# EasyVision-Ton/VMG

Measured on AMD Instinct MI355X. Metric: LR-frames/s (train: forward+loss+backward+AdamW), VMG-REDS-few_levels 4x SR, higher is better.
Workload: dtype bf16; 1 GPU; VMG-REDS-few_levels train step, per-GPU batch 4x7x3x64x64 -> 4x SR (BASELINE configs[1]); global_batch=4, frames_per_clip=7, parallelism=dp1, launch=eager, recompute_chains=False, fp8_chains=False

## Files before the change

include/vmg_hip.h:

```cpp
#ifndef VMG_HIP_H
#define VMG_HIP_H

#include <stdint.h>

#ifdef __cplusplus
extern "C" {
#endif

#define VMG_F32 0
#define VMG_BF16 1

#define VMG_ACT_NONE 0
#define VMG_ACT_RELU 1
#define VMG_ACT_LRELU 2
#define VMG_ACT_GELU 3

#define VMG_CONV_GENERAL 0
#define VMG_CONV_KSPLIT 2
#define VMG_CONV_WS 3
#define VMG_CONV_LINEAR_WRES 4
#define VMG_CONV_WSTAT 6

const char* vmg_last_error(void);
int vmg_version(void);
// ... 150 lines not shown
                       int B, int D, int H, int W, int C, int heads, int wt, int sd, int sh, int sw, void* stream);
int64_t vmg_win3d_attn_bwd_ws_bytes(int B, int D, int H, int W, int heads, int wt);
int vmg_win3d_attn_bwd(int dtype, const void* q, const void* kv, const float* bq, const float* bkv, const float* table, const void* out,
                       const float* lse, const void* d_out, void* dq, void* dkv, float* dtable, float* dbq, float* dbkv, void* ws, int B, int D, int H, int W,
                       int C, int heads, int wt, int sd, int sh, int sw, void* stream);
int vmg_win3d_variant(int variant);

int vmg_maxpool_fwd(int dtype, const void* x, void* y, unsigned char* idx, int N, int H, int W, int C, int f, void* stream);
int vmg_maxpool_bwd(int dtype, const void* dy, const unsigned char* idx, void* dx, int N, int H, int W, int C, int f, void* stream);

int vmg_se_mlp_fwd(const float* m, const float* w1, const float* b1, const float* w2, const float* b2, float* pre, float* out, int G, int C,
                   int Hd, int Co, int act1, int mode, void* stream);
int vmg_se_mlp_bwd(const float* dout, const float* out, const float* m, const float* pre, const float* w1, const float* w2, float* dm,
                   float* dw1, float* db1, float* dw2, float* db2, float* ws, int G, int C, int Hd, int Co, int act1, int mode, float dm_scale,
                   int accumulate, void* stream);

int vmg_avgpool2_nhwc(int dtype, const void* x, void* y, int n, int h, int w, int c, void* stream);
int vmg_upsample2x_ac_fwd(const float* x, float* y, int n, int h, int w, int c, float scale, void* stream);
int vmg_upsample2x_ac_bwd(const float* dy, float* dx, int n, int h, int w, int c, float scale, void* stream);
int vmg_spy_operand_fwd(int dtype, const void* ref, const void* warped, const float* up, void* out, int64_t npix, void* stream);
int vmg_spy_operand_bwd(int dtype, const void* dx8, void* dwarped, float* dup, int64_t npix, void* stream);
int vmg_spy_flow_add(int dtype, const float* up, const void* res, float* out, int64_t n, void* stream);
int vmg_spy_prep(int dtype, const float* img, const float* mean, const float* stdv, void* out, int64_t n, int h, int w, void* stream);

int vmg_tile_accumulate(int dtype, const void* patch, float* E, float* Wt, int64_t planes, int ph, int pw, int EH, int EW, int oh, int ow,
                        int top, int bottom, int left, int right, void* stream);
int vmg_tile_finalize(const float* E, const float* Wt, float* out_f32, unsigned char* out_u8, int64_t n, void* stream);

int64_t vmg_frame_metrics_ws_bytes(int T, int H, int W);
int vmg_frame_metrics(const unsigned char* a, const int64_t* a_strides, const unsigned char* b, const int64_t* b_strides, int T, int H, int W,
// ... 54 lines not shown
```

vmg_amd/csrc/tab_ops.hip:

```cpp
#include "common.h"

namespace {

template <typename T>
struct V16 {
  static constexpr int N = 16 / sizeof(T);
  T v[N];
};

template <typename T, int VN>
__global__ __launch_bounds__(256) void group_reduce_kernel(const T* __restrict__ a, const T* __restrict__ b, const T* __restrict__ c3,
                                                           float* __restrict__ out, int G, long long R, int C, int mode, float scale,
                                                           int chunks) {
  struct alignas(sizeof(T) * VN) Vec { T v[VN]; };
  __shared__ float red[VN * 256];
  const int g = blockIdx.x / chunks, ck = blockIdx.x - g * chunks;
  const int tpr = C / VN;
  const int rpb = 256 / tpr;
  const int roff = threadIdx.x / tpr, cp = threadIdx.x - roff * tpr;
  const long long r0 = R * ck / chunks, r1 = R * (ck + 1) / chunks;
  float s[VN];
#pragma unroll
  for (int e = 0; e < VN; ++e) s[e] = 0.f;
  if (roff < rpb) {
    const long long base = (long long)g * R * C + VN * cp;
    constexpr int U = 4;
    for (long long r = r0 + roff; r < r1; r += (long long)U * rpb) {
      Vec va[U], vb[U], vc[U];
      bool ok[U];
#pragma unroll
      for (int u = 0; u < U; ++u) {
// ... 22 lines not shown
#pragma unroll
          for (int e = 0; e < VN; ++e) s[e] += to_f32(va[u].v[e]) * to_f32(vb[u].v[e]);
        }
      }
    }
  }
#pragma unroll
  for (int e = 0; e < VN; ++e) red[e * 256 + threadIdx.x] = s[e];
  __syncthreads();
  for (int c = threadIdx.x; c < C; c += 256) {
    const int cp2 = c / VN, e = c - cp2 * VN;
    float t = 0.f;
    for (int k = 0; k < rpb; ++k) t += red[e * 256 + k * tpr + cp2];
    out[((long long)g * chunks + ck) * C + c] = t;
  }
}

__global__ __launch_bounds__(256) void group_reduce_final_kernel(const float* __restrict__ partial, float* __restrict__ out, int G, int chunks, int width,
                                                                 float scale) {
  __shared__ float sm[16][17];
  const int slabs = (width + 15) >> 4;
  const int g = blockIdx.x / slabs, c = (blockIdx.x - g * slabs) * 16 + (threadIdx.x & 15);
  const int q = threadIdx.x >> 4;
  float t = 0.f;
  if (c < width) {
    const float* p = partial + (long long)g * chunks * width + c;
#pragma unroll 4
    for (int k = q; k < chunks; k += 16) t += p[(long long)k * width];
  }
  sm[q][threadIdx.x & 15] = t;
  __syncthreads();
  if (q == 0 && c < width) {
    float u = 0.f;
#pragma unroll
    for (int i = 0; i < 16; ++i) u += sm[i][threadIdx.x & 15];
    out[(long long)g * width + c] = u * scale;
  }
}

template <typename T, int VN>
__global__ __launch_bounds__(256) void group_reduce3_kernel(const T* __restrict__ a, const T* __restrict__ b0, const T* __restrict__ b1,
                                                            const T* __restrict__ b2, float* __restrict__ out, int G, long long R, int C,
                                                            float scale, int chunks) {
  struct alignas(sizeof(T) * VN) Vec { T v[VN]; };
  __shared__ float red[3 * VN * 256];
  const int g = blockIdx.x / chunks, ck = blockIdx.x - g * chunks;
  const int tpr = C / VN;
  const int rpb = 256 / tpr;
  const int roff = threadIdx.x / tpr, cp = threadIdx.x - roff * tpr;
  const long long r0 = R * ck / chunks, r1 = R * (ck + 1) / chunks;
  float s[3][VN];
#pragma unroll
  for (int k = 0; k < 3; ++k)
#pragma unroll
    for (int e = 0; e < VN; ++e) s[k][e] = 0.f;
  if (roff < rpb) {
    const long long base = (long long)g * R * C + VN * cp;
    for (long long r = r0 + roff; r < r1; r += rpb) {
      const long long o = base + r * C;
      const Vec va = *reinterpret_cast<const Vec*>(a + o);
      const Vec v0 = *reinterpret_cast<const Vec*>(b0 + o), v1 = *reinterpret_cast<const Vec*>(b1 + o), v2 = *reinterpret_cast<const Vec*>(b2 + o);
// ... 6 lines not shown
      }
    }
  }
#pragma unroll
  for (int k = 0; k < 3; ++k)
#pragma unroll
    for (int e = 0; e < VN; ++e) red[(k * VN + e) * 256 + threadIdx.x] = s[k][e];
  __syncthreads();
  for (int i = threadIdx.x; i < 3 * C; i += 256) {
    const int c = i / 3, k = i - 3 * c;
    const int cp2 = c / VN, e = c - cp2 * VN;
    float t = 0.f;
    for (int j = 0; j < rpb; ++j) t += red[(k * VN + e) * 256 + j * tpr + cp2];
    out[(((long long)g * chunks + ck) * C + c) * 3 + k] = t;
  }
}

enum { OP_CA_FWD = 0, OP_CA_BWD = 1, OP_MIX_FWD = 2, OP_MIX_BWD = 3, OP_GATE_FWD = 4, OP_GATE_BWD = 5, OP_AFFINE2 = 6, OP_SCALE = 7, OP_GATE_RES_FWD = 8, OP_GATE_RES_BWD = 9 };

template <typename T>
__global__ __launch_bounds__(256) void tab_ew_kernel(int op, const T* __restrict__ p0, const T* __restrict__ p1, const T* __restrict__ p2,
                                                     const float* __restrict__ coef, const float* __restrict__ add, float s,
                                                     T* __restrict__ o0, T* __restrict__ o1, T* __restrict__ o2, long long rows,
                                                     long long R, int C) {
  constexpr int VN = V16<T>::N;
  const int nvec = C / VN;
  const long long total = rows * nvec;
  for (long long i = blockIdx.x * 256LL + threadIdx.x; i < total; i += (long long)gridDim.x * 256) {
    const long long row = i / nvec;
    const int v = (int)(i - row * nvec);
// ... 246 lines not shown
  } else if (i < n1 + n2) {
    const int e = i - n1, o = e / Hd, j = e - o * Hd;
    for (int g = 0; g < G; ++g) s += dz2[(long long)g * Co + o] * se_act(pre[g * Hd + j], act1);
    dw2[e] = accumulate ? dw2[e] + s : s;
  } else if (i < n1 + n2 + Hd) {
    const int j = i - n1 - n2;
    for (int g = 0; g < G; ++g) s += dz1[g * Hd + j];
    db1[j] = accumulate ? db1[j] + s : s;
  } else if (i < n1 + n2 + Hd + Co) {
    const int o = i - n1 - n2 - Hd;
    for (int g = 0; g < G; ++g) s += dz2[(long long)g * Co + o];
    db2[o] = accumulate ? db2[o] + s : s;
  }
}

}

extern "C" int vmg_se_mlp_fwd(const float* m, const float* w1, const float* b1, const float* w2, const float* b2, float* pre, float* out, int G,
                              int C, int Hd, int Co, int act1, int mode, void* stream) {
  VMG_CHECK(m && w1 && w2 && pre && out && G > 0 && C > 0 && Hd > 0 && Co > 0, "se_mlp_fwd: bad arguments");
  VMG_CHECK((act1 == 1 || act1 == 3) && (mode == 0 || (mode == 1 && Co % 3 == 0)), "se_mlp_fwd: act1 is ReLU (1) or GELU (3); mode 1 needs Co = 3 * channels");
  VMG_CHECK((C + Hd) * 4 <= 64 * 1024, "se_mlp_fwd: C + Hd too large");
  hipLaunchKernelGGL(se_mlp_fwd_kernel, dim3(G), dim3(1024), (C + Hd) * 4, (hipStream_t)stream, m, w1, b1, w2, b2, pre, out, C, Hd, Co, act1, mode);
  VMG_LAUNCH_CHECK();
  return 0;
}

extern "C" int vmg_se_mlp_bwd(const float* dout, const float* out, const float* m, const float* pre, const float* w1, const float* w2, float* dm,
                              float* dw1, float* db1, float* dw2, float* db2, float* ws, int G, int C, int Hd, int Co, int act1, int mode,
                              float dm_scale, int accumulate, void* stream) {
// ... 83 lines not shown
  const int chunks = gr_chunks(G, R);
  VMG_CHECK((int64_t)G * chunks * C * 3 * (int64_t)sizeof(float) <= ws_bytes, "group_reduce3: workspace too small (vmg_group_reduce_ws_bytes)");
  hipStream_t st = (hipStream_t)stream;
  if (dtype == VMG_BF16)
    hipLaunchKernelGGL((group_reduce3_kernel<bf16, 8>), dim3(G * chunks), dim3(256), 0, st, (const bf16*)a, (const bf16*)b0, (const bf16*)b1,
                       (const bf16*)b2, ws, G, (long long)R, C, scale, chunks);
  else
    hipLaunchKernelGGL((group_reduce3_kernel<float, 4>), dim3(G * chunks), dim3(256), 0, st, (const float*)a, (const float*)b0, (const float*)b1,
                       (const float*)b2, ws, G, (long long)R, C, scale, chunks);
  VMG_LAUNCH_CHECK();
  hipLaunchKernelGGL(group_reduce_final_kernel, dim3(G * cdiv(3 * C, 16)), dim3(256), 0, st, (const float*)ws, out, G, chunks, 3 * C, scale);
  VMG_LAUNCH_CHECK();
  return 0;
}

extern "C" int vmg_tab_elementwise(int dtype, int op, const void* p0, const void* p1, const void* p2, const float* coef, const float* add,
                                   float s, void* o0, void* o1, void* o2, int64_t rows, int64_t R, int C, void* stream) {
  VMG_CHECK(dtype == VMG_F32 || dtype == VMG_BF16, "tab_elementwise: bad dtype");
  VMG_CHECK(op >= 0 && op <= 9 && p0 && o0 && rows > 0 && R > 0 && C > 0, "tab_elementwise: bad arguments");
  const int vn = dtype == VMG_BF16 ? 8 : 4;
  VMG_CHECK(C % vn == 0, "tab_elementwise: C must be a multiple of %d", vn);
  const long long total = rows * (C / vn);
  const int blocks = (int)(cdiv64(total, 256) > 8192 ? 8192 : cdiv64(total, 256));
  hipStream_t st = (hipStream_t)stream;
  if (dtype == VMG_BF16)
    hipLaunchKernelGGL(tab_ew_kernel<bf16>, dim3(blocks), dim3(256), 0, st, op, (const bf16*)p0, (const bf16*)p1, (const bf16*)p2, coef, add, s,
                       (bf16*)o0, (bf16*)o1, (bf16*)o2, (long long)rows, (long long)R, C);
  else
    hipLaunchKernelGGL(tab_ew_kernel<float>, dim3(blocks), dim3(256), 0, st, op, (const float*)p0, (const float*)p1, (const float*)p2, coef, add,
                       s, (float*)o0, (float*)o1, (float*)o2, (long long)rows, (long long)R, C);
// ... 4 lines not shown
```

vmg_amd/functional.py:

```python
from __future__ import annotations

from typing import List, Optional, Sequence

import torch

from . import hip
from . import kernels as K
from .hip import HipError

class _Fn(torch.autograd.Function):

    @classmethod
    def apply(cls, *args):
        return super(torch.autograd.Function, cls).apply(*args)


def _pad_to(n: int, m: int = 8) -> int:
    return (n + m - 1) // m * m


def choose_tiling(M: int, cout: int, ks: int, dtype: torch.dtype, src_ch: Optional[Sequence[int]] = None, pixel_shuffle: bool = False):
    if USE_WS and src_ch is not None and not pixel_shuffle:
        t = K.ws_eligible(cout, ks, dtype, src_ch)
        if t and M <= 16384 and cout in (112, 144):
# ... 57 lines not shown
            if planned and hit[0][1] == ver[1] and key not in self.volatile:
                self.volatile.add(key)
                self.stamp += 1
        ent = [ver, build(key, weight, buf), weight]
        if planned and key not in self.volatile and _from_param(ent):
            self.stamp += 1
        ents[key] = ent
        return ent[1]

    def clear(self):
        self.ents.clear()
        self.q8.clear()
        self.volatile.clear()
        self.decay = None
        self.stamp += 1

    def bump_epoch(self):
        self.epoch += 1

    def settled(self, since: int, with_repack: bool) -> bool:
        return self.stamp == since and self.vol.stamp == since and (not with_repack or self.stable.stamp == since)

    def _run_plan(self, st: _PlanState, wkey, member, reset_sig: bool = False):
        fresh = st.stamp != self.stamp or st.wkey != wkey
        if fresh:
            st.ents = [ent for key, ent in self.ents.items() if member(key, ent)]
            st.packs, st.stamp, st.wkey = [ent[1] for ent in st.ents], self.stamp, wkey
            if reset_sig:
                st.plan.sig = None
        if not st.packs:
# ... 1016 lines not shown
        axis, chunk, Cp, shape = ctx.cfg
        return K.morph_tokens_gather(g.contiguous(), axis, chunk, Cp, Cp), None, None, None, None


def morph_linear(x: torch.Tensor, weight: torch.Tensor, bias: Optional[torch.Tensor], axis: str, chunk: int, Cp: int) -> torch.Tensor:
    if K.morph_fused_ok(x, chunk, Cp):
        return _MorphLinear.apply(x, weight, bias, axis, chunk, Cp)
    tok = _MorphGather.apply(x, axis, chunk, Cp)
    if tok.shape[-1] != Cp:
        padded, tok = tok, tok[:, :Cp]
        tok._vmg_padded = padded
    t = linear(tok, weight, bias, act=hip.ACT_RELU, alpha=1.0 / Cp)
    return _MorphScatter.apply(t, axis, chunk, Cp, tuple(x.shape))


class _ChannelAttention(_Fn):

    @staticmethod
    def forward(ctx, r, x, w1, b1, w2, b2, s):
        r, x = r.contiguous(), x.contiguous()
        N, C = r.shape[0], r.shape[-1]
        R = r.numel() // (N * C)
        m = K.group_reduce(r, N, scale=1.0 / R)
        pre, g = K.se_mlp_forward(m, w1.flatten(1), b1, w2.flatten(1), b2, hip.ACT_RELU, 0)
        out = K.tab_elementwise(K.OP_CA_FWD, r, x, coef=g, s=s, G=N)
        ctx.s, ctx.R = s, R
        ctx.save_for_backward(r, g, m, pre, w1, w2)
        DEFERRED.claim(ctx, w1, b1, w2, b2)
        return out

    @staticmethod
    def backward(ctx, dy):
        r, g, m, pre, w1, w2 = ctx.saved_tensors
        s, R = ctx.s, ctx.R
        dy = dy.contiguous()
        N = r.shape[0]
        dg = K.group_reduce(dy, N, b=r, mode=1, scale=s)
        dm, dw1, db1, dw2, db2 = K.se_mlp_backward(dg, g, m, pre, w1.flatten(1), w2.flatten(1), hip.ACT_RELU, 0, 1.0 / R, into=DEFERRED.into(ctx))
        d_r, d_x = K.tab_elementwise(K.OP_CA_BWD, dy, coef=g, add=dm, s=s, G=N, nout=2)
        DEFERRED.done(ctx)
        if ctx.direct:
            return d_r, d_x, None, None, None, None, None
        return (d_r, d_x, dw1.reshape(w1.shape), db1, dw2.reshape(w2.shape), db2, None)


def channel_attention_residual(r, x, w1, b1, w2, b2, out_scale: float):
    return _ChannelAttention.apply(r, x, w1, b1, w2, b2, float(out_scale))

class _ResidualDropPath(_Fn):

    @staticmethod
    def forward(ctx, res, y, g, gb=None):
        out = K.tab_elementwise(K.OP_CA_FWD, y.contiguous(), res.contiguous(), coef=g, s=1.0, G=g.shape[0])
# ... 66 lines not shown
            mask.div_(keep)
        g = (mask * scale).expand(B, C).contiguous()
    else:
        g = torch.full((B, C), float(scale), dtype=torch.float32, device=y.device)
    return _ResidualDropPath.apply(res, y, g)



class _ReweightMix(_Fn):

    @staticmethod
    def forward(ctx, h, w, c, fc1w, fc1b, fc2w, fc2b):
        h, w, c = h.contiguous(), w.contiguous(), c.contiguous()
        B, C = h.shape[0], h.shape[-1]
        R = h.numel() // (B * C)
        m = K.group_reduce(h, B, b=w, c3=c, scale=1.0 / R)
        pre, a = K.se_mlp_forward(m, fc1w, fc1b, fc2w, fc2b, hip.ACT_GELU, 1)
        y = K.tab_elementwise(K.OP_MIX_FWD, h, w, c, coef=a, G=B)
        ctx.R = R
        ctx.save_for_backward(h, w, c, a, m, pre, fc1w, fc2w)
        DEFERRED.claim(ctx, fc1w, fc1b, fc2w, fc2b)
        return y

    @staticmethod
    def backward(ctx, dy):
        h, w, c, a, m, pre, fc1w, fc2w = ctx.saved_tensors
        R = ctx.R
        dy = dy.contiguous()
        B, C = h.shape[0], h.shape[-1]
        da = K.group_reduce3(dy, h, w, c, B).reshape(B, 3 * C)
        dm, dw1, db1, dw2, db2 = K.se_mlp_backward(da, a, m, pre, fc1w, fc2w, hip.ACT_GELU, 1, 1.0 / R, into=DEFERRED.into(ctx))
        dh, dw, dc = K.tab_elementwise(K.OP_MIX_BWD, dy, coef=a, add=dm, G=B, nout=3)
        DEFERRED.done(ctx)
        if ctx.direct:
            return dh, dw, dc, None, None, None, None
        return dh, dw, dc, dw1, db1, dw2, db2


def reweight_mix(h, w, c, fc1w, fc1b, fc2w, fc2b):
    return _ReweightMix.apply(h, w, c, fc1w, fc1b, fc2w, fc2b)


class _TanhGate(_Fn):

    @staticmethod
    def forward(ctx, x, y):
# ... 352 lines not shown
```

vmg_amd/hip.py:

```python
from __future__ import annotations

import ctypes
import os
from ctypes import POINTER, c_char_p, c_float, c_int, c_int64, c_void_p

import torch

HERE = os.path.dirname(os.path.abspath(__file__))
LIB_PATH = os.environ.get("VMG_HIP_LIB") or os.path.join(HERE, "libvmg_hip.so")

F32, BF16 = 0, 1
ACT_NONE, ACT_RELU, ACT_LRELU, ACT_GELU = 0, 1, 2, 3
CONV_GENERAL, CONV_KSPLIT, CONV_WS, CONV_LINEAR_WRES, CONV_WSTAT = 0, 2, 3, 4, 6


class HipError(RuntimeError):
    pass


class ConvDesc(ctypes.Structure):
    _fields_ = [
        ("dtype", c_int), ("ks", c_int), ("cout_tiles", c_int),
        ("N", c_int), ("H", c_int), ("W", c_int), ("Cout", c_int),
        ("nsrc", c_int),
# ... 79 lines not shown
    "vmg_win3d_variant": (c_int, [c_int]),
    "vmg_linear_wgrad2_multi": (c_int, [c_int, c_int, c_void_p, c_void_p, c_int64, c_int64, c_int, c_int64, c_int, c_void_p, c_int, c_int, c_int,
                                        c_void_p, c_void_p, c_void_p, c_int64, c_void_p]),
    "vmg_replay_build": (c_void_p, [c_void_p, c_void_p, c_void_p]),
    "vmg_replay_kernel_info": (c_int, [c_void_p, c_int, c_void_p, c_void_p, c_void_p, c_void_p]),
    "vmg_replay_run": (c_int, [c_void_p, c_int, c_int, c_void_p]),
    "vmg_replay_destroy": (None, [c_void_p]),
    "vmg_pack_entry_bytes": (c_int, []),
    "vmg_pack_entry": (c_int, [c_void_p, c_int, c_int, c_void_p, c_int, c_int, c_int, c_int, c_int, c_int, c_void_p, c_void_p, c_int, c_int, c_void_p,
                               c_int]),
    "vmg_pack_run": (c_int, [c_void_p, c_int, c_int, c_void_p]),
    "vmg_group_reduce3": (c_int, [c_int, c_void_p, c_void_p, c_void_p, c_void_p, c_void_p, c_int, c_int64, c_int, ctypes.c_float, c_void_p, c_int64, c_void_p]),
    "vmg_group_reduce_ws_bytes": (c_int64, []),
    "vmg_se_mlp_fwd": (c_int, [c_void_p] * 7 + [c_int] * 6 + [c_void_p]),
    "vmg_se_mlp_bwd": (c_int, [c_void_p] * 12 + [c_int] * 6 + [ctypes.c_float, c_int, c_void_p]),
    "vmg_maxpool_fwd": (c_int, [c_int, c_void_p, c_void_p, c_void_p, c_int, c_int, c_int, c_int, c_int, c_void_p]),
    "vmg_maxpool_bwd": (c_int, [c_int, c_void_p, c_void_p, c_void_p, c_int, c_int, c_int, c_int, c_int, c_void_p]),
    "vmg_avgpool2_nhwc": (c_int, [c_int, c_void_p, c_void_p, c_int, c_int, c_int, c_int, c_void_p]),
    "vmg_upsample2x_ac_fwd": (c_int, [c_void_p, c_void_p, c_int, c_int, c_int, c_int, c_float, c_void_p]),
    "vmg_upsample2x_ac_bwd": (c_int, [c_void_p, c_void_p, c_int, c_int, c_int, c_int, c_float, c_void_p]),
    "vmg_spy_operand_fwd": (c_int, [c_int, c_void_p, c_void_p, c_void_p, c_void_p, c_int64, c_void_p]),
    "vmg_spy_operand_bwd": (c_int, [c_int, c_void_p, c_void_p, c_void_p, c_int64, c_void_p]),
    "vmg_spy_flow_add": (c_int, [c_int, c_void_p, c_void_p, c_void_p, c_int64, c_void_p]),
    "vmg_spy_prep": (c_int, [c_int, c_void_p, c_void_p, c_void_p, c_void_p, c_int64, c_int, c_int, c_void_p]),
    "vmg_space_depth_ln_fwd": (c_int, [c_int, c_int, c_void_p, c_void_p, c_void_p, c_void_p, c_void_p, c_void_p, c_int, c_int, c_int, c_int, c_float, c_void_p]),
    "vmg_space_depth_ln_bwd": (c_int, [c_int, c_int, c_void_p, c_void_p, c_void_p, c_void_p, c_void_p, c_void_p, c_void_p, c_void_p, c_int, c_int, c_int, c_int,
                                       c_void_p, c_void_p]),
    "vmg_conv_wgrad_batched": (c_int, [c_int, c_int, c_int, POINTER(c_void_p), POINTER(c_void_p), c_int, c_int, c_int, c_int64, c_int,
                                       c_int64, c_int, c_void_p, c_int, c_int, c_int, c_void_p, c_float, c_void_p]),
    "vmg_warp_bilinear_fwd": (c_int, [c_int, c_void_p, c_void_p, c_void_p, c_int, c_int, c_int, c_int, c_void_p]),
# ... 110 lines not shown
```

vmg_amd/kernels.py:

```python
from __future__ import annotations

import ctypes
import os
import struct
from typing import Optional, Sequence, Tuple

import torch

from . import hip
from .hip import ConvDesc, HipError


def _intarr(v: Sequence[int]):
    return (ctypes.c_int * len(v))(*[int(x) for x in v])


def cout_tiles_for(cout: int, dtype: torch.dtype = torch.bfloat16, ks: int = 3) -> int:
    t = (cout + 15) // 16
    if t <= 1:
        return 1
    if ks == 7:
        return 2 if t == 2 else 4
    if t <= 4:
        return 4
# ... 996 lines not shown
        dm, ws = parts
        dw1, db1, dw2, db2 = into
        for t, n in zip(into, (Hd * C, Hd, Co * Hd, Co)):
            if t.dtype != torch.float32 or not t.is_contiguous() or t.numel() != n or not t.is_cuda:
                raise HipError("se_mlp: gradient buffers must be contiguous fp32 of the parameters' sizes")
    else:
        dm, ws, dw1, db1, dw2, db2 = parts
    hip.check(hip.lib().vmg_se_mlp_bwd(dout.data_ptr(), out.data_ptr(), m.data_ptr(), pre.data_ptr(), w1.data_ptr(), w2.data_ptr(), dm.data_ptr(),
                                       dw1.data_ptr(), db1.data_ptr(), dw2.data_ptr(), db2.data_ptr(), ws.data_ptr(), G, C, Hd, Co, act1, mode,
                                       float(dm_scale), 1 if into is not None else 0, hip.stream_ptr()), "vmg_se_mlp_bwd")
    if into is not None:
        return dm.view(G, C), dw1, db1, dw2, db2
    return dm.view(G, C), dw1.view(Hd, C), db1, dw2.view(Co, Hd), db2


class PackPlan:

    def __init__(self):
        self.sig, self.dev, self.n, self.blocks = None, None, 0, 0
        self.retired = []

    def run(self, packs: Sequence[PackedConv], reuse: bool = False):
        l = hip.lib()
        if reuse and self.sig is not None:
            hip.check(l.vmg_pack_run(self.dev.data_ptr(), self.n, self.blocks, hip.stream_ptr()), "vmg_pack_run")
            return
        packs = [p for p in packs if p.call is not None]
        if not packs:
            return
        sig = tuple((p.call[0], p.buf.data_ptr()) for p in packs)
# ... 153 lines not shown
```

Before: 599.4 LR-frames/s.

## Fuse pooled group reduction with SE-style gate MLP via last-block ticket

Adds fused forward and backward kernels that do the per-group pooled reduction and then, in the last-arriving workgroup per group (selected with an atomic ticket counter), finalize the reduction and run the small gate MLP. Backward also computes dm and, in a globally last workgroup, the weight and bias gradients. The aim is to replace several small kernel launches (reduce, final reduce, MLP fwd/bwd) with one launch per direction. The cost is serialized MLP work on one workgroup, plus atomics and fences that rely on the workspace counters being zeroed correctly.

```diff
diff --git a/include/vmg_hip.h b/include/vmg_hip.h
--- a/include/vmg_hip.h
+++ b/include/vmg_hip.h
@@ -188,6 +188,15 @@
 int vmg_se_mlp_bwd(const float* dout, const float* out, const float* m, const float* pre, const float* w1, const float* w2, float* dm,
                    float* dw1, float* db1, float* dw2, float* db2, float* ws, int G, int C, int Hd, int Co, int act1, int mode, float dm_scale,
                    int accumulate, void* stream);
+int64_t vmg_pooled_gate_ws_bytes(void);
+int64_t vmg_pooled_gate_counter_bytes(void);
+int vmg_pooled_gate_fwd(int dtype, const void* a, const void* b, const void* c3, const float* w1, const float* b1, const float* w2,
+                        const float* b2, float* m, float* pre, float* gate, int G, int64_t R, int C, int Hd, int Co, int act1, int mode,
+                        float scale, void* ws, int64_t ws_bytes, void* stream);
+int vmg_pooled_gate_bwd(int dtype, const void* dy, const void* b0, const void* b1, const void* b2, const float* gate, const float* m,
+                        const float* pre, const float* w1, const float* w2, float* dm, float* dw1, float* db1, float* dw2, float* db2,
+                        float* dz, int G, int64_t R, int C, int Hd, int Co, int act1, int mode, float scale, float dm_scale, int accumulate,
+                        void* ws, int64_t ws_bytes, void* stream);
 
 int vmg_avgpool2_nhwc(int dtype, const void* x, void* y, int n, int h, int w, int c, void* stream);
 int vmg_upsample2x_ac_fwd(const float* x, float* y, int n, int h, int w, int c, float scale, void* stream);
diff --git a/vmg_amd/csrc/tab_ops.hip b/vmg_amd/csrc/tab_ops.hip
--- a/vmg_amd/csrc/tab_ops.hip
+++ b/vmg_amd/csrc/tab_ops.hip
@@ -9,12 +9,10 @@
 };
 
 template <typename T, int VN>
-__global__ __launch_bounds__(256) void group_reduce_kernel(const T* __restrict__ a, const T* __restrict__ b, const T* __restrict__ c3,
-                                                           float* __restrict__ out, int G, long long R, int C, int mode, float scale,
-                                                           int chunks) {
+__device__ __forceinline__ void group_reduce_block(const T* __restrict__ a, const T* __restrict__ b, const T* __restrict__ c3,
+                                                   float* __restrict__ out, long long R, int C, int mode, int chunks, int g, int ck,
+                                                   float* __restrict__ red ) {
   struct alignas(sizeof(T) * VN) Vec { T v[VN]; };
-  __shared__ float red[VN * 256];
-  const int g = blockIdx.x / chunks, ck = blockIdx.x - g * chunks;
   const int tpr = C / VN;
   const int rpb = 256 / tpr;
   const int roff = threadIdx.x / tpr, cp = threadIdx.x - roff * tpr;
@@ -67,6 +65,15 @@
     for (int k = 0; k < rpb; ++k) t += red[e * 256 + k * tpr + cp2];
     out[((long long)g * chunks + ck) * C + c] = t;
   }
+}
+
+template <typename T, int VN>
+__global__ __launch_bounds__(256) void group_reduce_kernel(const T* __restrict__ a, const T* __restrict__ b, const T* __restrict__ c3,
+                                                           float* __restrict__ out, int G, long long R, int C, int mode, float scale,
+                                                           int chunks) {
+  __shared__ float red[VN * 256];
+  const int g = blockIdx.x / chunks, ck = blockIdx.x - g * chunks;
+  group_reduce_block<T, VN>(a, b, c3, out, R, C, mode, chunks, g, ck, red);
 }
 
 __global__ __launch_bounds__(256) void group_reduce_final_kernel(const float* __restrict__ partial, float* __restrict__ out, int G, int chunks, int width,
@@ -92,12 +99,10 @@
 }
 
 template <typename T, int VN>
-__global__ __launch_bounds__(256) void group_reduce3_kernel(const T* __restrict__ a, const T* __restrict__ b0, const T* __restrict__ b1,
-                                                            const T* __restrict__ b2, float* __restrict__ out, int G, long long R, int C,
-                                                            float scale, int chunks) {
+__device__ __forceinline__ void group_reduce3_block(const T* __restrict__ a, const T* __restrict__ b0, const T* __restrict__ b1,
+                                                    const T* __restrict__ b2, float* __restrict__ out, long long R, int C, int chunks, int g,
+                                                    int ck, float* __restrict__ red ) {
   struct alignas(sizeof(T) * VN) Vec { T v[VN]; };
-  __shared__ float red[3 * VN * 256];
-  const int g = blockIdx.x / chunks, ck = blockIdx.x - g * chunks;
   const int tpr = C / VN;
   const int rpb = 256 / tpr;
   const int roff = threadIdx.x / tpr, cp = threadIdx.x - roff * tpr;
@@ -134,6 +139,15 @@
     for (int j = 0; j < rpb; ++j) t += red[(k * VN + e) * 256 + j * tpr + cp2];
     out[(((long long)g * chunks + ck) * C + c) * 3 + k] = t;
   }
+}
+
+template <typename T, int VN>
+__global__ __launch_bounds__(256) void group_reduce3_kernel(const T* __restrict__ a, const T* __restrict__ b0, const T* __restrict__ b1,
+                                                            const T* __restrict__ b2, float* __restrict__ out, int G, long long R, int C,
+                                                            float scale, int chunks) {
+  __shared__ float red[3 * VN * 256];
+  const int g = blockIdx.x / chunks, ck = blockIdx.x - g * chunks;
+  group_reduce3_block<T, VN>(a, b0, b1, b2, out, R, C, chunks, g, ck, red);
 }
 
 enum { OP_CA_FWD = 0, OP_CA_BWD = 1, OP_MIX_FWD = 2, OP_MIX_BWD = 3, OP_GATE_FWD = 4, OP_GATE_BWD = 5, OP_AFFINE2 = 6, OP_SCALE = 7, OP_GATE_RES_FWD = 8, OP_GATE_RES_BWD = 9 };
@@ -410,6 +424,229 @@
   }
 }
 
+constexpr int PG_COUNTERS = 1024;
+constexpr int PG_FIN = 16 * 65;
+
+__device__ __forceinline__ bool pg_ticket(int* counter, int last) {
+  __shared__ int drew_last;
+  __threadfence();
+  __syncthreads();
+  if (threadIdx.x == 0) drew_last = atomicAdd(counter, 1) == last;
+  __syncthreads();
+  const bool r = drew_last != 0;
+  if (r) __threadfence();
+  return r;
+}
+
+__device__ __forceinline__ void pg_final(const float* part, int chunks, int width, float scale, float* fin, float* vec, float* outg) {
+  const int tid = threadIdx.x, q = tid >> 4, c4 = tid & 15;
+  for (int s0 = 0; s0 < width; s0 += 64) {
+    const int c = s0 + 4 * c4;
+    float t[4] = {0.f, 0.f, 0.f, 0.f};
+    if (c < width) {
+      for (int k0 = q; k0 < chunks; k0 += 128) {
+        float4 v[8];
+#pragma unroll
+        for (int u = 0; u < 8; ++u)
+          if (k0 + 16 * u < chunks) v[u] = *reinterpret_cast<const float4*>(part + (long long)(k0 + 16 * u) * width + c);
+#pragma unroll
+        for (int u = 0; u < 8; ++u)
+          if (k0 + 16 * u < chunks) { t[0] += v[u].x; t[1] += v[u].y; t[2] += v[u].z; t[3] += v[u].w; }
+      }
+    }
+#pragma unroll
+    for (int e = 0; e < 4; ++e) fin[q * 65 + 4 * c4 + e] = t[e];
+    __syncthreads();
+    if (tid < 64 && s0 + tid < width) {
+      float u = 0.f;
+#pragma unroll
+      for (int i = 0; i < 16; ++i) u += fin[i * 65 + tid];
+      u *= scale;
+      vec[s0 + tid] = u;
+      if (outg) outg[s0 + tid] = u;
+    }
+    __syncthreads();
+  }
+}
+
+template <typename F>
+__device__ __forceinline__ void pg_wave_dots(const float* x, int n, const float* __restrict__ W, int sx, int sj, int nj, F sink) {
+  constexpr int JB = 3, KM = 8;
+  const int lane = threadIdx.x & 63, wave = threadIdx.x >> 6;
+  for (int j0 = wave; j0 < nj; j0 += 4 * JB) {
+    float wv[JB][KM];
+#pragma unroll
+    for (int b = 0; b < JB; ++b)
+#pragma unroll
+      for (int k = 0; k < KM; ++k) {
+        const int j = j0 + 4 * b, i = lane + 64 * k;
+        wv[b][k] = (j < nj && i < n) ? W[(long long)i * sx + (long long)j * sj] : 0.f;
+      }
+#pragma unroll
+    for (int b = 0; b < JB; ++b) {
+      const int j = j0 + 4 * b;
+      if (j < nj) {
+        float s = 0.f;
+#pragma unroll
+        for (int k = 0; k < KM; ++k) {
+          const int i = lane + 64 * k;
+          if (i < n) s += wv[b][k] * x[i];
+        }
+        sink(j, wave_sum(s));
+      }
+    }
+  }
+}
+
+__device__ __forceinline__ void pg_mlp_fwd_row(int g, const float* mrow, float* z1, const float* __restrict__ w1, const float* __restrict__ b1,
+                                               const float* __restrict__ w2, const float* __restrict__ b2, float* __restrict__ pre,
+                                               float* __restrict__ out, int C, int Hd, int Co, int act1, int mode) {
+  const int tid = threadIdx.x;
+  pg_wave_dots(mrow, C, w1, 1, C, Hd, [&](int j, float s) {
+    s = s + (b1 ? b1[j] : 0.f);
+    if ((tid & 63) == 0) { pre[(long long)g * Hd + j] = s; z1[j] = se_act(s, act1); }
+  });
+  __syncthreads();
+  if (mode == 0) {
+    for (int o = tid; o < Co; o += 256) {
+      float s = b2 ? b2[o] : 0.f;
+      const float* wr = w2 + (long long)o * Hd;
+#pragma unroll 12
+      for (int j = 0; j < Hd; ++j) s += wr[j] * z1[j];
+      out[(long long)g * Co + o] = 1.f / (1.f + expf(-s));
+    }
+  } else {
+    for (int c = tid; c < Co / 3; c += 256) {
+      float z[3];
+      const float* wr = w2 + (long long)3 * c * Hd;
+#pragma unroll
+      for (int k = 0; k < 3; ++k) z[k] = b2 ? b2[3 * c + k] : 0.f;
+#pragma unroll 12
+      for (int j = 0; j < Hd; ++j) {
+#pragma unroll
+        for (int k = 0; k < 3; ++k) z[k] += wr[k * Hd + j] * z1[j];
+      }
+      const float mx = fmaxf(z[0], fmaxf(z[1], z[2]));
+      const float e0 = expf(z[0] - mx), e1 = expf(z[1] - mx), e2 = expf(z[2] - mx), inv = 1.f / (e0 + e1 + e2);
+      float* orow = out + (long long)g * Co + 3 * c;
+      orow[0] = e0 * inv; orow[1] = e1 * inv; orow[2] = e2 * inv;
+    }
+  }
+}
+
+struct PgMlp {
+  const float *w1, *b1, *w2, *b2;
+  float *m, *pre, *gate;
+  float *dm, *dw1, *db1, *dw2, *db2, *dz;
+  int Hd, Co, act1, mode, accumulate;
+  float dm_scale;
+};
+
+template <typename T, int VN>
+__global__ __launch_bounds__(256) void pooled_gate_fwd_kernel(const T* __restrict__ a, const T* __restrict__ b, const T* __restrict__ c3, int* cnt,
+                                                              float* part, long long R, int C, float scale, int chunks, int rmode, PgMlp p) {
+  extern __shared__ float4 pg_smem[];
+  float* lds = reinterpret_cast<float*>(pg_smem);
+  const int g = blockIdx.x / chunks, ck = blockIdx.x - g * chunks;
+  group_reduce_block<T, VN>(a, b, c3, part, R, C, rmode, chunks, g, ck, lds);
+  if (!pg_ticket(cnt + g, chunks - 1)) return;
+  float* fin = lds;
+  float* mrow = lds + PG_FIN;
+  float* z1 = mrow + C;
+  pg_final(part + (long long)g * chunks * C, chunks, C, scale, fin, mrow, p.m + (long long)g * C);
+  pg_mlp_fwd_row(g, mrow, z1, p.w1, p.b1, p.w2, p.b2, p.pre, p.gate, C, p.Hd, p.Co, p.act1, p.mode);
+  if (threadIdx.x == 0) cnt[g] = 0;
+}
+
+template <typename T, int VN, bool THREE>
+__global__ __launch_bounds__(256) void pooled_gate_bwd_kernel(const T* __restrict__ dy, const T* __restrict__ b0, const T* __restrict__ b1,
+                                                              const T* __restrict__ b2, int* cnt, float* part, int G, long long R, int C,
+                                                              float scale, int chunks, int rmode, PgMlp p) {
+  extern __shared__ float4 pg_smem[];
+  float* lds = reinterpret_cast<float*>(pg_smem);
+  const int g = blockIdx.x / chunks, ck = blockIdx.x - g * chunks, tid = threadIdx.x;
+  const int Hd = p.Hd, Co = p.Co;
+  if (THREE) group_reduce3_block<T, VN>(dy, b0, b1, b2, part, R, C, chunks, g, ck, lds);
+  else group_reduce_block<T, VN>(dy, b0, (const T*)nullptr, part, R, C, rmode, chunks, g, ck, lds);
+  if (!pg_ticket(cnt + g, chunks - 1)) return;
+  {
+    float* fin = lds;
+    float* drow = lds + PG_FIN;
+    float* dz2 = drow + Co;
+    float* dz1 = dz2 + Co;
+    pg_final(part + (long long)g * chunks * Co, chunks, Co, scale, fin, drow, nullptr);
+    float* gz2 = p.dz + (long long)g * Co;
+    float* gz1 = p.dz + (long long)G * Co + (long long)g * Hd;
+    const float* orow = p.gate + (long long)g * Co;
+    if (p.mode == 0) {
+      for (int o = tid; o < Co; o += 256) { const float v = drow[o] * orow[o] * (1.f - orow[o]); dz2[o] = v; gz2[o] = v; }
+    } else {
+      for (int c = tid; c < Co / 3; c += 256) {
+        const float a0 = orow[3 * c], a1 = orow[3 * c + 1], a2 = orow[3 * c + 2];
+        const float d0 = drow[3 * c], d1 = drow[3 * c + 1], d2 = drow[3 * c + 2];
+        const float sd = a0 * d0 + a1 * d1 + a2 * d2;
+        const float v0 = a0 * (d0 - sd), v1 = a1 * (d1 - sd), v2 = a2 * (d2 - sd);
+        dz2[3 * c] = v0; dz2[3 * c + 1] = v1; dz2[3 * c + 2] = v2;
+        gz2[3 * c] = v0; gz2[3 * c + 1] = v1; gz2[3 * c + 2] = v2;
+      }
+    }
+    __syncthreads();
+    pg_wave_dots(dz2, Co, p.w2, Hd, 1, Hd, [&](int j, float s) {
+      s = s * se_dact(p.pre[(long long)g * Hd + j], p.act1);
+      if ((tid & 63) == 0) { dz1[j] = s; gz1[j] = s; }
+    });
+    __syncthreads();
+    for (int c = tid; c < C; c += 256) {
+      float s = 0.f;
+#pragma unroll 12
+      for (int j = 0; j < Hd; ++j) s += dz1[j] * p.w1[(long long)j * C + c];
+      p.dm[(long long)g * C + c] = s * p.dm_scale;
+    }
+    if (tid == 0) cnt[g] = 0;
+  }
+  if (!pg_ticket(cnt + PG_COUNTERS - 1, G - 1)) return;
+  float* dz2 = lds;
+  float* dz1 = dz2 + (long long)G * Co;
+  float* ms = dz1 + G * Hd;
+  float* z1 = ms + G * C;
+  for (int i = tid; i < G * (Co + Hd); i += 256) lds[i] = p.dz[i];
+  for (int i = tid; i < G * C; i += 256) ms[i] = p.m[i];
+  for (int i = tid; i < G * Hd; i += 256) z1[i] = se_act(p.pre[i], p.act1);
+  __syncthreads();
+  const int n1 = Hd * C, n2 = Co * Hd, total = n1 + n2 + Hd + Co;
+  for (int i0 = tid; i0 < total; i0 += 4 * 256) {
+    float* dst[4];
+    float old[4];
+#pragma unroll
+    for (int u = 0; u < 4; ++u) {
+      const int i = i0 + 256 * u;
+      dst[u] = i >= total ? nullptr : i < n1 ? p.dw1 + i : i < n1 + n2 ? p.dw2 + (i - n1) : i < n1 + n2 + Hd ? p.db1 + (i - n1 - n2) : p.db2 + (i - n1 - n2 - Hd);
+      old[u] = (dst[u] && p.accumulate) ? *dst[u] : 0.f;
+    }
+#pragma unroll
+    for (int u = 0; u < 4; ++u) {
+      const int i = i0 + 256 * u;
+      if (!dst[u]) continue;
+      float s = 0.f;
+      if (i < n1) {
+        const int j = i / C, c = i - j * C;
+        for (int r = 0; r < G; ++r) s += dz1[r * Hd + j] * ms[r * C + c];
+      } else if (i < n1 + n2) {
+        const int e = i - n1, o = e / Hd, j = e - o * Hd;
+        for (int r = 0; r < G; ++r) s += dz2[r * Co + o] * z1[r * Hd + j];
+      } else if (i < n1 + n2 + Hd) {
+        const int j = i - n1 - n2;
+        for (int r = 0; r < G; ++r) s += dz1[r * Hd + j];
+      } else {
+        const int o = i - n1 - n2 - Hd;
+        for (int r = 0; r < G; ++r) s += dz2[r * Co + o];
+      }
+      *dst[u] = p.accumulate ? old[u] + s : s;
+    }
+  }
+  if (tid == 0) cnt[PG_COUNTERS - 1] = 0;
+}
+
 }
 
 extern "C" int vmg_se_mlp_fwd(const float* m, const float* w1, const float* b1, const float* w2, const float* b2, float* pre, float* out, int G,
@@ -523,6 +760,74 @@
   return 0;
 }
 
+extern "C" int64_t vmg_pooled_gate_counter_bytes() { return (int64_t)PG_COUNTERS * sizeof(int); }
+extern "C" int64_t vmg_pooled_gate_ws_bytes() { return vmg_pooled_gate_counter_bytes() + vmg_group_reduce_ws_bytes(); }
+
+static int pg_check(const char* who, int dtype, int G, int64_t R, int C, int Hd, int Co, int act1, int mode, const void* ws, int64_t ws_bytes,
+                    int chunks, int64_t lds_floats) {
+  VMG_CHECK(dtype == VMG_F32 || dtype == VMG_BF16, "%s: bad dtype", who);
+  VMG_CHECK(G > 0 && G < PG_COUNTERS && R > 0 && Hd > 0 && C > 0 && C <= 512 && C % (dtype == VMG_BF16 ? 8 : 4) == 0, "%s: bad shape (G < %d, C <= 512 in whole 16-byte vectors)", who, PG_COUNTERS);
+  VMG_CHECK((act1 == 1 || act1 == 3) && ((mode == 0 && Co == C) || (mode == 1 && Co == 3 * C)), "%s: ReLU (1) / GELU (3); Co = C (sigmoid) or 3 C (softmax)", who);
+  VMG_CHECK(Co <= 512, "%s: at most 512 gate values per row", who);
+  VMG_CHECK(ws && (uintptr_t)ws % 16 == 0 && vmg_pooled_gate_counter_bytes() + (int64_t)G * chunks * Co * (int64_t)sizeof(float) <= ws_bytes, "%s: workspace too small (vmg_pooled_gate_ws_bytes)", who);
+  VMG_CHECK(lds_floats * 4 <= 64 * 1024, "%s: the rows do not fit the last workgroup's LDS", who);
+  return 0;
+}
+
+extern "C" int vmg_pooled_gate_fwd(int dtype, const void* a, const void* b, const void* c3, const float* w1, const float* b1, const float* w2,
+                                   const float* b2, float* m, float* pre, float* gate, int G, int64_t R, int C, int Hd, int Co, int act1, int mode,
+                                   float scale, void* ws, int64_t ws_bytes, void* stream) {
+  VMG_CHECK(a && w1 && w2 && m && pre && gate && (b || !c3), "pooled_gate_fwd: bad arguments");
+  VMG_CHECK((((uintptr_t)a | (uintptr_t)b | (uintptr_t)c3) % 16) == 0, "pooled_gate_fwd: pointers must be 16-byte aligned");
+  const int chunks = gr_chunks(G, R);
+  const int vn = dtype == VMG_BF16 ? 8 : 4;
+  const int64_t tail = PG_FIN + C + Hd, lds = tail > vn * 256 ? tail : vn * 256;
+  if (int e = pg_check("pooled_gate_fwd", dtype, G, R, C, Hd, Co, act1, mode, ws, ws_bytes, chunks, lds)) return e;
+  VMG_CHECK((int64_t)G * chunks * C * (int64_t)sizeof(float) + vmg_pooled_gate_counter_bytes() <= ws_bytes, "pooled_gate_fwd: workspace too small");
+  PgMlp p = {};
+  p.w1 = w1; p.b1 = b1; p.w2 = w2; p.b2 = b2; p.m = m; p.pre = pre; p.gate = gate; p.Hd = Hd; p.Co = Co; p.act1 = act1; p.mode = mode;
+  int* cnt = (int*)ws;
+  float* part = (float*)((char*)ws + vmg_pooled_gate_counter_bytes());
+  hipStream_t st = (hipStream_t)stream;
+  if (dtype == VMG_BF16)
+    hipLaunchKernelGGL((pooled_gate_fwd_kernel<bf16, 8>), dim3(G * chunks), dim3(256), lds * 4, st, (const bf16*)a, (const bf16*)b, (const bf16*)c3, cnt,
+                       part, (long long)R, C, scale, chunks, 0, p);
+  else
+    hipLaunchKernelGGL((pooled_gate_fwd_kernel<float, 4>), dim3(G * chunks), dim3(256), lds * 4, st, (const float*)a, (const float*)b, (const float*)c3,
+                       cnt, part, (long long)R, C, scale, chunks, 0, p);
+  VMG_LAUNCH_CHECK();
+  return 0;
+}
+
+extern "C" int vmg_pooled_gate_bwd(int dtype, const void* dy, const void* b0, const void* b1, const void* b2, const float* gate, const float* m,
+                                   const float* pre, const float* w1, const float* w2, float* dm, float* dw1, float* db1, float* dw2, float* db2,
+                                   float* dz, int G, int64_t R, int C, int Hd, int Co, int act1, int mode, float scale, float dm_scale, int accumulate,
+                                   void* ws, int64_t ws_bytes, void* stream) {
+  VMG_CHECK(dy && b0 && gate && m && pre && w1 && w2 && dm && dw1 && db1 && dw2 && db2 && dz && (mode == 0 || (b1 && b2)), "pooled_gate_bwd: bad arguments");
+  VMG_CHECK((((uintptr_t)dy | (uintptr_t)b0 | (uintptr_t)b1 | (uintptr_t)b2) % 16) == 0, "pooled_gate_bwd: pointers must be 16-byte aligned");
+  const int chunks = gr_chunks(G, R);
+  const int vn = dtype == VMG_BF16 ? 8 : 4;
+  int64_t lds = (mode == 1 ? 3 : 1) * vn * 256;
+  if (lds < PG_FIN + 2 * Co + Hd) lds = PG_FIN + 2 * Co + Hd;
+  if (lds < (int64_t)G * (Co + 2 * Hd + C)) lds = (int64_t)G * (Co + 2 * Hd + C);
+  if (int e = pg_check("pooled_gate_bwd", dtype, G, R, C, Hd, Co, act1, mode, ws, ws_bytes, chunks, lds)) return e;
+  PgMlp p = {};
+  p.w1 = w1; p.w2 = w2; p.m = const_cast<float*>(m); p.pre = const_cast<float*>(pre); p.gate = const_cast<float*>(gate);
+  p.dm = dm; p.dw1 = dw1; p.db1 = db1; p.dw2 = dw2; p.db2 = db2; p.dz = dz;
+  p.Hd = Hd; p.Co = Co; p.act1 = act1; p.mode = mode; p.accumulate = accumulate; p.dm_scale = dm_scale;
+  int* cnt = (int*)ws;
+  float* part = (float*)((char*)ws + vmg_pooled_gate_counter_bytes());
+  hipStream_t st = (hipStream_t)stream;
+#define PG_BWD(T, VN, THREE)                                                                                                                     \
+  hipLaunchKernelGGL((pooled_gate_bwd_kernel<T, VN, THREE>), dim3(G * chunks), dim3(256), lds * 4, st, (const T*)dy, (const T*)b0, (const T*)b1, \
+                     (const T*)b2, cnt, part, G, (long long)R, C, scale, chunks, 1, p)
+  if (dtype == VMG_BF16) { if (mode == 1) PG_BWD(bf16, 8, true); else PG_BWD(bf16, 8, false); }
+  else { if (mode == 1) PG_BWD(float, 4, true); else PG_BWD(float, 4, false); }
+#undef PG_BWD
+  VMG_LAUNCH_CHECK();
+  return 0;
+}
+
 extern "C" int vmg_tab_elementwise(int dtype, int op, const void* p0, const void* p1, const void* p2, const float* coef, const float* add,
                                    float s, void* o0, void* o1, void* o2, int64_t rows, int64_t R, int C, void* stream) {
   VMG_CHECK(dtype == VMG_F32 || dtype == VMG_BF16, "tab_elementwise: bad dtype");
diff --git a/vmg_amd/functional.py b/vmg_amd/functional.py
--- a/vmg_amd/functional.py
+++ b/vmg_amd/functional.py
@@ -95,6 +95,7 @@
         self.volatile.clear()
         self.decay = None
         self.stamp += 1
+        K.release_pooled_gate_workspace()
 
     def bump_epoch(self):
         self.epoch += 1
@@ -1141,6 +1142,9 @@
     return _MorphScatter.apply(t, axis, chunk, Cp, tuple(x.shape))
 
 
+POOLED_GATE_FUSED = False
+
+
 class _ChannelAttention(_Fn):
 
     @staticmethod
@@ -1148,8 +1152,11 @@
         r, x = r.contiguous(), x.contiguous()
         N, C = r.shape[0], r.shape[-1]
         R = r.numel() // (N * C)
-        m = K.group_reduce(r, N, scale=1.0 / R)
-        pre, g = K.se_mlp_forward(m, w1.flatten(1), b1, w2.flatten(1), b2, hip.ACT_RELU, 0)
+        if POOLED_GATE_FUSED and K.pooled_gate_ok(r, N, w1.shape[0], 0):
+            m, pre, g = K.pooled_gate_forward(r, N, w1.flatten(1), b1, w2.flatten(1), b2, hip.ACT_RELU, 0, scale=1.0 / R)
+        else:
+            m = K.group_reduce(r, N, scale=1.0 / R)
+            pre, g = K.se_mlp_forward(m, w1.flatten(1), b1, w2.flatten(1), b2, hip.ACT_RELU, 0)
         out = K.tab_elementwise(K.OP_CA_FWD, r, x, coef=g, s=s, G=N)
         ctx.s, ctx.R = s, R
         ctx.save_for_backward(r, g, m, pre, w1, w2)
@@ -1162,8 +1169,12 @@
         s, R = ctx.s, ctx.R
         dy = dy.contiguous()
         N = r.shape[0]
-        dg = K.group_reduce(dy, N, b=r, mode=1, scale=s)
-        dm, dw1, db1, dw2, db2 = K.se_mlp_backward(dg, g, m, pre, w1.flatten(1), w2.flatten(1), hip.ACT_RELU, 0, 1.0 / R, into=DEFERRED.into(ctx))
+        if POOLED_GATE_FUSED and K.pooled_gate_ok(dy, N, w1.shape[0], 0):
+            dm, dw1, db1, dw2, db2 = K.pooled_gate_backward(dy, (r,), N, g, m, pre, w1.flatten(1), w2.flatten(1), hip.ACT_RELU, 0, s, 1.0 / R,
+                                                            into=DEFERRED.into(ctx))
+        else:
+            dg = K.group_reduce(dy, N, b=r, mode=1, scale=s)
+            dm, dw1, db1, dw2, db2 = K.se_mlp_backward(dg, g, m, pre, w1.flatten(1), w2.flatten(1), hip.ACT_RELU, 0, 1.0 / R, into=DEFERRED.into(ctx))
         d_r, d_x = K.tab_elementwise(K.OP_CA_BWD, dy, coef=g, add=dm, s=s, G=N, nout=2)
         DEFERRED.done(ctx)
         if ctx.direct:
@@ -1260,8 +1271,11 @@
         h, w, c = h.contiguous(), w.contiguous(), c.contiguous()
         B, C = h.shape[0], h.shape[-1]
         R = h.numel() // (B * C)
-        m = K.group_reduce(h, B, b=w, c3=c, scale=1.0 / R)
-        pre, a = K.se_mlp_forward(m, fc1w, fc1b, fc2w, fc2b, hip.ACT_GELU, 1)
+        if POOLED_GATE_FUSED and K.pooled_gate_ok(h, B, fc1w.shape[0], 1):
+            m, pre, a = K.pooled_gate_forward(h, B, fc1w, fc1b, fc2w, fc2b, hip.ACT_GELU, 1, b=w, c3=c, scale=1.0 / R)
+        else:
+            m = K.group_reduce(h, B, b=w, c3=c, scale=1.0 / R)
+            pre, a = K.se_mlp_forward(m, fc1w, fc1b, fc2w, fc2b, hip.ACT_GELU, 1)
         y = K.tab_elementwise(K.OP_MIX_FWD, h, w, c, coef=a, G=B)
         ctx.R = R
         ctx.save_for_backward(h, w, c, a, m, pre, fc1w, fc2w)
@@ -1274,8 +1288,11 @@
         R = ctx.R
         dy = dy.contiguous()
         B, C = h.shape[0], h.shape[-1]
-        da = K.group_reduce3(dy, h, w, c, B).reshape(B, 3 * C)
-        dm, dw1, db1, dw2, db2 = K.se_mlp_backward(da, a, m, pre, fc1w, fc2w, hip.ACT_GELU, 1, 1.0 / R, into=DEFERRED.into(ctx))
+        if POOLED_GATE_FUSED and K.pooled_gate_ok(dy, B, fc1w.shape[0], 1):
+            dm, dw1, db1, dw2, db2 = K.pooled_gate_backward(dy, (h, w, c), B, a, m, pre, fc1w, fc2w, hip.ACT_GELU, 1, 1.0, 1.0 / R, into=DEFERRED.into(ctx))
+        else:
+            da = K.group_reduce3(dy, h, w, c, B).reshape(B, 3 * C)
+            dm, dw1, db1, dw2, db2 = K.se_mlp_backward(da, a, m, pre, fc1w, fc2w, hip.ACT_GELU, 1, 1.0 / R, into=DEFERRED.into(ctx))
         dh, dw, dc = K.tab_elementwise(K.OP_MIX_BWD, dy, coef=a, add=dm, G=B, nout=3)
         DEFERRED.done(ctx)
         if ctx.direct:
diff --git a/vmg_amd/hip.py b/vmg_amd/hip.py
--- a/vmg_amd/hip.py
+++ b/vmg_amd/hip.py
@@ -117,6 +117,11 @@
     "vmg_group_reduce_ws_bytes": (c_int64, []),
     "vmg_se_mlp_fwd": (c_int, [c_void_p] * 7 + [c_int] * 6 + [c_void_p]),
     "vmg_se_mlp_bwd": (c_int, [c_void_p] * 12 + [c_int] * 6 + [ctypes.c_float, c_int, c_void_p]),
+    "vmg_pooled_gate_ws_bytes": (c_int64, []),
+    "vmg_pooled_gate_counter_bytes": (c_int64, []),
+    "vmg_pooled_gate_fwd": (c_int, [c_int] + [c_void_p] * 10 + [c_int, c_int64] + [c_int] * 5 + [ctypes.c_float, c_void_p, c_int64, c_void_p]),
+    "vmg_pooled_gate_bwd": (c_int, [c_int] + [c_void_p] * 15 + [c_int, c_int64] + [c_int] * 5 + [ctypes.c_float, ctypes.c_float, c_int, c_void_p, c_int64,
+                                                                                                   c_void_p]),
     "vmg_maxpool_fwd": (c_int, [c_int, c_void_p, c_void_p, c_void_p, c_int, c_int, c_int, c_int, c_int, c_void_p]),
     "vmg_maxpool_bwd": (c_int, [c_int, c_void_p, c_void_p, c_void_p, c_int, c_int, c_int, c_int, c_int, c_void_p]),
     "vmg_avgpool2_nhwc": (c_int, [c_int, c_void_p, c_void_p, c_int, c_int, c_int, c_int, c_void_p]),
diff --git a/vmg_amd/kernels.py b/vmg_amd/kernels.py
--- a/vmg_amd/kernels.py
+++ b/vmg_amd/kernels.py
@@ -1034,6 +1034,101 @@
     return dm.view(G, C), dw1.view(Hd, C), db1, dw2.view(Co, Hd), db2
 
 
+def _pooled_gate_workspace(device) -> Optional[torch.Tensor]:
+    ws = _WS.get(("vmg_pooled_gate_ws_bytes", device))
+    if ws is None and not torch.cuda.is_current_stream_capturing():
+        ws = _workspace("vmg_pooled_gate_ws_bytes", device, zero=True)
+    return ws
+
+
+def release_pooled_gate_workspace():
+    for key in [k for k in _WS if k[0] == "vmg_pooled_gate_ws_bytes"]:
+        del _WS[key]
+
+
+def pooled_gate_ok(a: torch.Tensor, G: int, Hd: int, mode: int) -> bool:
+    C = a.shape[-1]
+    Co = 3 * C if mode == 1 else C
+    vec = 8 if a.dtype == torch.bfloat16 else 4
+    if a.dtype not in (torch.bfloat16, torch.float32) or C % vec or Co > 512 or not 0 < G < 1024 or a.data_ptr() % 16:
+        return False
+    if max(G * (C + Co + 2 * Hd), 16 * 65 + 2 * Co + Hd, (3 if mode == 1 else 1) * vec * 256) * 4 > 64 * 1024:
+        return False
+    return _pooled_gate_workspace(a.device) is not None
+
+
+def _pg_operands(who: str, G: int, first: torch.Tensor, *rest):
+    C = first.shape[-1]
+    rows = first.numel() // C
+    if rows % G or any(t is not None and (t.shape != first.shape or t.dtype != first.dtype or not t.is_contiguous()) for t in (first, *rest)):
+        raise HipError(who + ": contiguous tensors of one shape / dtype covering G groups expected")
+    return rows // G, C
+
+
+def pooled_gate_forward(a: torch.Tensor, G: int, w1: torch.Tensor, b1, w2: torch.Tensor, b2, act1: int, mode: int,
+                        b: Optional[torch.Tensor] = None, c3: Optional[torch.Tensor] = None, scale: float = 1.0, ws: Optional[torch.Tensor] = None):
+    hip.require_cuda(a, b, c3, w1, w2)
+    R, C = _pg_operands("pooled_gate_forward", G, a, b, c3)
+    Hd, Co = w1.shape[0], w2.shape[0]
+    for t in (w1, w2, b1, b2):
+        if t is not None and (t.dtype != torch.float32 or not t.is_contiguous()):
+            raise HipError("pooled_gate: contiguous fp32 parameters only")
+    if w1.numel() != Hd * C or w2.numel() != Co * Hd:
+        raise HipError("pooled_gate: w1 (Hd, C) and w2 (Co, Hd) expected")
+    ws = ws if ws is not None else _pooled_gate_workspace(a.device)
+    if ws is None:
+        raise HipError("pooled_gate: no workspace (first use inside a stream capture)")
+    m = torch.empty(G, C, dtype=torch.float32, device=a.device)
+    pre = torch.empty(G, Hd, dtype=torch.float32, device=a.device)
+    gate = torch.empty(G, Co, dtype=torch.float32, device=a.device)
+    ptr = lambda t: t.data_ptr() if t is not None else None
+    hip.check(hip.lib().vmg_pooled_gate_fwd(hip.dtype_code(a.dtype), a.data_ptr(), ptr(b), ptr(c3), w1.data_ptr(), ptr(b1), w2.data_ptr(), ptr(b2),
+                                            m.data_ptr(), pre.data_ptr(), gate.data_ptr(), G, R, C, Hd, Co, act1, mode, float(scale), ws.data_ptr(),
+                                            ws.numel(), hip.stream_ptr()), "vmg_pooled_gate_fwd")
+    return m, pre, gate
+
+
+def pooled_gate_backward(dy: torch.Tensor, ops: Sequence[torch.Tensor], G: int, gate: torch.Tensor, m: torch.Tensor, pre: torch.Tensor,
+                         w1: torch.Tensor, w2: torch.Tensor, act1: int, mode: int, scale: float, dm_scale: float, into=None,
+                         ws: Optional[torch.Tensor] = None):
+    hip.require_cuda(dy, *ops, gate, m, pre, w1, w2)
+    if len(ops) != (3 if mode == 1 else 1):
+        raise HipError("pooled_gate_backward: one operand (sigmoid gate) or three (softmax weights) expected")
+    R, C = _pg_operands("pooled_gate_backward", G, dy, *ops)
+    Hd, Co = w1.shape[0], w2.shape[0]
+    for t in (gate, m, pre, w1, w2):
+        if t.dtype != torch.float32 or not t.is_contiguous():
+            raise HipError("pooled_gate: contiguous fp32 tensors only")
+    if m.numel() != G * C or pre.numel() != G * Hd or gate.numel() != G * Co or w1.numel() != Hd * C or w2.numel() != Co * Hd:
+        raise HipError("pooled_gate_backward: m (G, C), pre (G, Hd), gate (G, Co), w1 (Hd, C), w2 (Co, Hd) expected")
+    ws = ws if ws is not None else _pooled_gate_workspace(dy.device)
+    if ws is None:
+        raise HipError("pooled_gate: no workspace (first use inside a stream capture)")
+    sizes = (G * C, G * (Co + Hd)) if into is not None else (G * C, G * (Co + Hd), Hd * C, Hd, Co * Hd, Co)
+    buf = torch.empty(sum(sizes), dtype=torch.float32, device=dy.device)
+    parts, o = [], 0
+    for n in sizes:
+        parts.append(buf[o:o + n])
+        o += n
+    if into is not None:
+        dm, dz = parts
+        dw1, db1, dw2, db2 = into
+        for t, n in zip(into, (Hd * C, Hd, Co * Hd, Co)):
+            if t.dtype != torch.float32 or not t.is_contiguous() or t.numel() != n or not t.is_cuda:
+                raise HipError("pooled_gate: gradient buffers must be contiguous fp32 of the parameters' sizes")
+    else:
+        dm, dz, dw1, db1, dw2, db2 = parts
+    b = list(ops) + [None] * (3 - len(ops))
+    ptr = lambda t: t.data_ptr() if t is not None else None
+    hip.check(hip.lib().vmg_pooled_gate_bwd(hip.dtype_code(dy.dtype), dy.data_ptr(), ptr(b[0]), ptr(b[1]), ptr(b[2]), gate.data_ptr(), m.data_ptr(),
+                                            pre.data_ptr(), w1.data_ptr(), w2.data_ptr(), dm.data_ptr(), dw1.data_ptr(), db1.data_ptr(),
+                                            dw2.data_ptr(), db2.data_ptr(), dz.data_ptr(), G, R, C, Hd, Co, act1, mode, float(scale), float(dm_scale),
+                                            1 if into is not None else 0, ws.data_ptr(), ws.numel(), hip.stream_ptr()), "vmg_pooled_gate_bwd")
+    if into is not None:
+        return dm.view(G, C), dw1, db1, dw2, db2
+    return dm.view(G, C), dw1.view(Hd, C), db1, dw2.view(Co, Hd), db2
+
+
 class PackPlan:
 
     def __init__(self):
```

Result: no change. 597.3 LR-frames/s, median of 2 (-0.4%).
